# al-mcintyre/mCaller

Measured on NVIDIA B200. Metric: per-read site calls/sec, higher is better.
Workload: dtype f64

## Files before the change

include/mcaller_b200.h:

```cpp
#ifndef MCALLER_B200_H
#define MCALLER_B200_H

#include <stdint.h>

#ifdef __cplusplus
extern "C" {
#endif

#define MC_ABI_VERSION 3

#define MC_TILE_BYTES 3840
#define MC_TEXT_PAD 4096
#define MC_MAXK 8

enum {
    MC_OK = 0,
    MC_EINVAL = -1,
    MC_ECUDA = -2,
    MC_ECAPACITY = -3
};

typedef struct mc_refindex {
    int32_t n_contigs;
    int32_t k;
// ... 50 lines not shown

typedef struct mc_call {
    int64_t read_off;
    double prob;
    double feat[MC_MAXK + 1];
    int32_t read_len;
    int32_t mpos;
    int32_t site;
    uint32_t close_rec;
    uint16_t win_contig;
    uint16_t chrom_contig;
    uint8_t kind;
    uint8_t rev;
    uint8_t n_empty;
    uint8_t empty_mask;
    uint8_t model_sel;
    uint8_t label;
    uint8_t err;
    uint8_t pad0;
    uint32_t seg;
    uint32_t pad1;
    uint32_t pad2;
} mc_call;

enum { MC_CALL = 0, MC_TOO_MANY_SKIPS = 1, MC_MULTI_M = 2, MC_NONE = 3  };
#define MC_CE_CONTEXT 1u
#define MC_CE_MODELKEY 2u
#define MC_CE_BADNUM 4u
#define MC_CE_COLUMN 8u
#define MC_CE_SPACING 16u

enum { MC_MLP = 0, MC_LR = 1, MC_GNB = 2, MC_RF = 3 };
enum { MC_ACT_IDENTITY = 0, MC_ACT_LOGISTIC = 1, MC_ACT_TANH = 2, MC_ACT_RELU = 3 };
typedef struct mc_model {
    int32_t kind;
    int32_t n_in;
    int32_t n_layers;
    int32_t hidden_act;
    int32_t sizes[8];
    const double *d_weights;
    const double *d_biases;
    int32_t n_trees;
    int32_t max_nodes;
    const int32_t *d_tree_off;
    const int32_t *d_left;
    const int32_t *d_right;
    const int32_t *d_feature;
    const double *d_threshold;
    const double *d_leaf_p1;
} mc_model;

typedef struct mc_qual_entry {
    uint64_t hash;
    uint32_t check;
    uint32_t len;
    double qual;
} mc_qual_entry;


int mc_version(void);
int mc_sizeof(int what);
const char *mc_last_error(void);

int mc_read_u64(const uint64_t *d_src, int64_t n, uint64_t *h_dst, void *stream);

int mc_scan(const uint8_t *d_text, int64_t nbytes, const mc_refindex *ref, int dense,
            mc_record *d_rec, int64_t rec_cap, uint32_t *d_tile_tab , uint32_t *d_run_tab ,
            uint64_t *d_counters, void *stream);

int mc_scan_run_len(int64_t nbytes);

int mc_scan_set_run_len(int run_len);

int64_t mc_num_tiles(int64_t nbytes);

int64_t mc_workspace_bytes(int64_t n);

int mc_order_records(const uint8_t *d_text, int64_t nbytes, const mc_refindex *ref, const uint32_t *d_tile_tab, int64_t n_tiles,
                     uint32_t *d_run_tab, int run_len, const mc_record *d_rec_in, int64_t rec_in_cap, const uint64_t *d_scan_counters,
                     mc_record *d_rec_out, int64_t rec_out_cap, uint64_t *d_n_out, uint32_t *d_seg_flags ,
                     uint32_t *d_run_first , void *d_ws, void *stream);

int mc_segment_reads(const uint8_t *d_text, mc_record *d_rec, const uint64_t *d_n_records, int64_t rec_cap,
                     uint32_t *d_seg_flags , const uint32_t *d_run_first, int64_t n_runs,
                     uint32_t *d_seg_start, uint64_t *d_nseg, void *d_ws, void *stream);

int mc_segment_quality(const uint8_t *d_text, const mc_record *d_rec, const uint32_t *d_seg_start, const uint64_t *d_nseg,
                       int64_t seg_cap, const mc_qual_entry *d_table, int64_t table_size, double *d_seg_qual, uint64_t *d_err,
                       void *stream);

int mc_build_windows(const mc_record *d_rec, const uint64_t *d_n_records, int64_t rec_cap, const uint32_t *d_seg_start,
                     const uint64_t *d_nseg, int64_t seg_cap, const double *d_seg_qual, const mc_refindex *ref, int skip_thresh,
                     double qual_thresh, int two_models, mc_call *d_calls, int64_t call_cap, uint32_t *d_seg_count,
                     uint64_t *d_ncalls, void *d_ws, double *d_spill, int64_t spill_cap, void *stream);

typedef struct mc_carry {
    mc_call row;
    uint32_t valid;
    int32_t first_kept_contig;
    uint64_t chunks;
    uint64_t pad[6];
} mc_carry;
int mc_carry_reset(mc_carry *d_carry, void *stream);
int mc_carry_rows(mc_call *d_rows, const uint64_t *d_ncalls, const mc_record *d_rec, const uint64_t *d_n_records,
                  const uint32_t *d_seg_start, const uint64_t *d_nseg, const double *d_seg_qual, double qual_thresh,
                  mc_carry *d_carry, uint64_t *d_nrows_out, const uint64_t *d_abort, void *stream);
int mc_chunk_guard(const uint64_t *d_counters, int64_t rec_cap, const uint64_t *d_n_records, int64_t rec_out_cap,
                   const uint64_t *d_nseg, int64_t seg_cap, const uint64_t *d_ncalls, int64_t call_cap, uint64_t *d_abort,
                   uint64_t *d_sticky , void *stream);
int mc_carry_close(mc_carry *d_carry, int closing_contig, const int64_t *d_next_contigs, int from, int count, mc_call *d_row_out,
                   uint32_t *d_depth, uint32_t *d_meth, uint64_t *d_first, int64_t n_sites, uint64_t *d_row_base, void *stream);

int64_t mc_classify_workspace_bytes(int64_t row_cap);
int mc_classify(mc_call *d_calls, const uint64_t *d_nrows, int64_t row_cap, const mc_model *models, void *d_ws, void *stream);

int mc_hist_accumulate(const mc_call *d_calls, const uint64_t *d_nrows, int64_t row_cap, uint32_t *d_depth, uint32_t *d_meth,
                       uint64_t *d_first, int64_t n_sites, uint64_t *d_row_base, mc_call *d_odd, int64_t odd_cap, uint64_t *d_n_odd,
                       const uint64_t *d_abort , void *stream);

int mc_bed_select(const uint32_t *d_depth, const uint32_t *d_meth, int64_t n_sites, int64_t depth_thresh, double mod_thresh,
                  int control, uint8_t *d_flags, uint64_t *d_count, void *stream);

int mc_count_calls(const mc_call *d_calls, const uint64_t *d_nrows, int64_t row_cap, uint64_t *d_out, void *stream);

typedef struct mc_locus_entry {
    unsigned long long hash;
    unsigned long long first_off;
    unsigned long long check;
    uint32_t depth;
    uint32_t meth;
} mc_locus_entry;

typedef struct mc_diffs_row {
    uint64_t line_off;
    uint32_t slot;
    uint32_t values_off;
    uint32_t values_len;
    uint32_t prob_off;
    uint32_t prob_len;
    uint32_t pad;
} mc_diffs_row;
int mc_diffs_aggregate_ex(const uint8_t *d_text, int64_t nbytes, int64_t base_off, const uint64_t *d_posset, int64_t posset_size,
                          mc_locus_entry *d_table, int64_t table_size, uint64_t *d_counters, void *stream);
int mc_diffs_rehash(const mc_locus_entry *d_old, int64_t old_size, mc_locus_entry *d_table, int64_t table_size,
                    uint64_t *d_counters, void *stream);
int mc_diffs_rows(const uint8_t *d_text, int64_t nbytes, const uint64_t *d_posset, int64_t posset_size,
                  const mc_locus_entry *d_table, int64_t table_size, mc_diffs_row *d_rows, int64_t row_cap, uint64_t *d_nrows,
                  void *stream);
int mc_diffs_colstats(const uint8_t *d_text, const mc_diffs_row *d_rows, const uint32_t *d_order, int64_t n_rows,
                      const uint32_t *d_locus_off, int64_t n_loci, int ncols, double *d_vals, uint32_t *d_ncol,
                      double *d_stats, uint64_t *d_counters, void *stream);

int64_t mc_format_rows(const mc_call *h_calls, int64_t n_calls, const uint8_t *h_text, const uint8_t *carry_name,
                       int32_t carry_name_len, const char *const *contig_names, const char *const *marked_fwd,
                       const char *const *marked_rev, const int64_t *contig_len, int32_t n_contigs, int32_t k,
                       const char *base_label, const char *mod_label, int32_t with_prob, int32_t max_threads, char *out,
                       int64_t out_cap);

int64_t mc_fastq_tiles(int64_t nbytes);
int mc_fastq_index(const uint8_t *d_text, int64_t nbytes, uint32_t *d_tile_cnt, uint32_t *d_tile_off, uint64_t *d_line_start,
                   int64_t line_cap, uint64_t *d_n_newlines, void *d_ws, void *stream);
int mc_fastq_quality(const uint8_t *d_text, int64_t nbytes, const uint64_t *d_line_start, int64_t n_lines, mc_qual_entry *d_table,
                     int64_t table_size, uint32_t *d_owner, double *d_rec_mean, uint64_t *d_stats, void *stream);

#define MC_TRAIN_HIDDEN 100
#define MC_TRAIN_BATCH 200
typedef struct mc_train_job {
// ... 42 lines not shown
```

mcaller_b200/csrc/records.cu:

```cuda
#include "parse.cuh"

namespace {

constexpr int SCAN_THREADS = 256;
constexpr int SCAN_IPT = 8;
constexpr int SCAN_BLOCK = SCAN_THREADS * SCAN_IPT;

__global__ void __launch_bounds__(SCAN_THREADS) k_scan_reduce(const uint32_t *__restrict__ in, int64_t n_cap,
                                                            const unsigned long long *__restrict__ d_n,
                                                            unsigned long long *__restrict__ block_sums) {
    __shared__ int s_warp[SCAN_THREADS / 32 + 1];
    const int64_t n = d_n ? mc_dev_count(d_n, n_cap) : n_cap;
    const int64_t base = (int64_t)blockIdx.x * SCAN_BLOCK;
    unsigned long long acc = 0ull;
#pragma unroll
    for (int j = 0; j < SCAN_IPT; ++j) {
        const int64_t i = base + (int64_t)j * SCAN_THREADS + threadIdx.x;
        if (i < n) acc += in[i];
    }
    for (int d = 16; d > 0; d >>= 1) acc += __shfl_down_sync(0xffffffffu, acc, d);
    __shared__ unsigned long long s_sum[SCAN_THREADS / 32];
    if ((threadIdx.x & 31) == 0) s_sum[threadIdx.x >> 5] = acc;
    __syncthreads();
    if (threadIdx.x == 0) {
// ... 13 lines not shown
    const int lane = threadIdx.x & 31, wid = threadIdx.x >> 5;
    for (int64_t c0 = 0; c0 < nb; c0 += 1024) {
        const int64_t i = c0 + threadIdx.x;
        const unsigned long long v = (i < nb) ? block_sums[i] : 0ull;
        unsigned long long inc = v;
        for (int d = 1; d < 32; d <<= 1) {
            unsigned long long t = __shfl_up_sync(0xffffffffu, inc, d);
            if (lane >= d) inc += t;
        }
        if (lane == 31) s_w[wid] = inc;
        __syncthreads();
        if (wid == 0) {
            unsigned long long x = s_w[lane], xi = x;
            for (int d = 1; d < 32; d <<= 1) {
                unsigned long long t = __shfl_up_sync(0xffffffffu, xi, d);
                if (lane >= d) xi += t;
            }
            s_w[lane] = xi - x;
            if (lane == 31) s_w[32] = xi;
        }
        __syncthreads();
        const unsigned long long carry = s_carry;
        if (i < nb) block_sums[i] = carry + s_w[wid] + inc - v;
        __syncthreads();
        if (threadIdx.x == 0) s_carry = carry + s_w[32];
        __syncthreads();
    }
    if (threadIdx.x == 0 && d_total) *d_total = s_carry;
}

__global__ void __launch_bounds__(SCAN_THREADS) k_scan_down(const uint32_t *__restrict__ in, int64_t n_cap,
                                                          const unsigned long long *__restrict__ d_n,
                                                          const unsigned long long *__restrict__ block_sums,
                                                          uint32_t *__restrict__ out) {
    __shared__ int s_warp[SCAN_THREADS / 32 + 1];
    const int64_t n = d_n ? mc_dev_count(d_n, n_cap) : n_cap;
    if ((int64_t)blockIdx.x * SCAN_BLOCK >= n) return;
    const int64_t base = (int64_t)blockIdx.x * SCAN_BLOCK + (int64_t)threadIdx.x * SCAN_IPT;
    uint32_t v[SCAN_IPT];
    int sum = 0;
#pragma unroll
    for (int j = 0; j < SCAN_IPT; ++j) {
        const int64_t i = base + j;
        v[j] = (i < n) ? in[i] : 0u;
        sum += (int)v[j];
    }
    int total;
    int off = mc_block_exscan<SCAN_THREADS>(sum, s_warp, total);
    uint32_t run = (uint32_t)block_sums[blockIdx.x] + (uint32_t)off;
#pragma unroll
    for (int j = 0; j < SCAN_IPT; ++j) {
        const int64_t i = base + j;
        if (i < n) out[i] = run;
        run += v[j];
    }
}

}

int64_t mc_exscan_ws_bytes(int64_t n) { return ((n + SCAN_BLOCK - 1) / SCAN_BLOCK + 1) * 8 + 256; }

int mc_exscan_u32(const uint32_t *d_in, uint32_t *d_out, int64_t n_cap, const uint64_t *d_n, uint64_t *d_total, void *d_ws,
                  cudaStream_t st) {
    if (n_cap <= 0) {
        if (d_total) MC_CUDA_CHECK(cudaMemsetAsync(d_total, 0, 8, st));
        return MC_OK;
    }
    const int64_t nb = (n_cap + SCAN_BLOCK - 1) / SCAN_BLOCK;
    unsigned long long *sums = reinterpret_cast<unsigned long long *>(d_ws);
    const unsigned long long *dn = reinterpret_cast<const unsigned long long *>(d_n);
    k_scan_reduce<<<(unsigned)nb, SCAN_THREADS, 0, st>>>(d_in, n_cap, dn, sums);
    MC_LAUNCH_CHECK();
    k_scan_sums<<<1, 1024, 0, st>>>(sums, nb, reinterpret_cast<unsigned long long *>(d_total));
    MC_LAUNCH_CHECK();
    k_scan_down<<<(unsigned)nb, SCAN_THREADS, 0, st>>>(d_in, n_cap, dn, sums, d_out);
    MC_LAUNCH_CHECK();
    return MC_OK;
}

extern "C" int64_t mc_windows_workspace_bytes(int64_t rec_cap);
extern "C" int64_t mc_workspace_bytes(int64_t n) {
    if (n < 1) n = 1;
    const int64_t a = ((n * 4 + 255) / 256) * 256;
    const int64_t mine = 2 * a + mc_exscan_ws_bytes(n) + 512;
    const int64_t win = mc_windows_workspace_bytes(n);
    return mine > win ? mine : win;
}
static inline uint32_t *ws_a(void *ws) { return reinterpret_cast<uint32_t *>(ws); }
static inline uint32_t *ws_b(void *ws, int64_t n) { return reinterpret_cast<uint32_t *>(reinterpret_cast<uint8_t *>(ws) + ((n * 4 + 255) / 256) * 256); }
static inline void *ws_s(void *ws, int64_t n) { return reinterpret_cast<uint8_t *>(ws) + 2 * (((n * 4 + 255) / 256) * 256); }

namespace {

__global__ void __launch_bounds__(256) k_run_resolve(uint32_t *__restrict__ run_tab, int64_t n_runs, uint32_t *__restrict__ cnt_clean,
                                                    const unsigned long long *__restrict__ scan_counters, unsigned long long rec_in_cap) {
    const int64_t r = (int64_t)blockIdx.x * blockDim.x + threadIdx.x;
    if (r >= n_runs) return;
    if (scan_counters && (scan_counters[MC_C_OVERFLOW] != 0ull || scan_counters[MC_C_RECORDS] > rec_in_cap)) {
        cnt_clean[r] = 0u;
        return;
    }
    uint32_t count = run_tab[2 * r];
    const uint32_t v = run_tab[2 * r + 1];
    if (v & 1u) {
        int64_t p = r - 1;
        uint32_t st = 0u;
        while (p >= 0 && (st = (run_tab[2 * p + 1] >> 1) & 3u) == 0u) --p;
        if (p >= 0 && st == 1u && count > 0u) {
            run_tab[2 * r + 1] = v | 0x80000000u;
            --count;
        }
    }
    cnt_clean[r] = count;
}

__global__ void __launch_bounds__(256, 4) k_gather_finish(const uint8_t *__restrict__ text, int64_t limit, mc_refindex R,
                                                      const uint32_t *__restrict__ tile_tab, const uint32_t *__restrict__ run_tab,
                                                      const uint32_t *__restrict__ run_dst, int64_t n_tiles, int64_t n_runs, int run_len,
                                                      const mc_record *__restrict__ in, unsigned long long in_cap, mc_record *__restrict__ out,
                                                      unsigned long long out_cap, uint32_t *__restrict__ seg_flags,
                                                      uint32_t *__restrict__ run_first) {
    const int lane = threadIdx.x & 31;
    const int64_t warp0 = ((int64_t)blockIdx.x * blockDim.x + threadIdx.x) >> 5, n_warps = ((int64_t)gridDim.x * blockDim.x) >> 5;
    for (int64_t run = warp0; run < n_runs; run += n_warps) {
    const uint32_t rv = __ldg(run_tab + 2 * run + 1);
    const bool empty_run = __ldg(run_dst + run) == __ldg(run_dst + run + 1);
    if (run_first && lane == 0) run_first[run] = empty_run ? 0xFFFFFFFFu : __ldg(run_dst + run);
    if (__ldg(run_tab + 2 * run) == 0u) continue;
    const bool drop = (rv >> 31) != 0u;
    unsigned long long d_run = __ldg(run_dst + run);
    const int64_t c0 = run * run_len, c1 = min(c0 + (int64_t)run_len, n_tiles);
    long long carry_line = -1;
    uint32_t carry_span = 0u;
    for (int64_t cb = c0; cb < c1; cb += 32) {
        const int64_t c = cb + lane;
        unsigned long long src = 0ull;
        uint32_t cnt = 0u;
        if (c < c1) {
            const uint2 e = __ldg(reinterpret_cast<const uint2 *>(tile_tab) + c);
            src = e.x;
            cnt = e.y & 0xFFFFu;
            if (drop && ((e.y >> 16) & 1u) && cnt > 0u) { src += 1ull; --cnt; }
        }
        uint32_t incl = cnt;
#pragma unroll
        for (int d = 1; d < 32; d <<= 1) {
            const uint32_t t = __shfl_up_sync(0xffffffffu, incl, d);
            if (lane >= d) incl += t;
        }
        const uint32_t excl = incl - cnt, tot = __shfl_sync(0xffffffffu, incl, 31);
        for (uint32_t k0 = 0; k0 < tot; k0 += 32) {
            const uint32_t idx = k0 + lane;
            const bool act = idx < tot;
            int lo = 0, hi = 31;
#pragma unroll
            for (int st = 0; st < 5; ++st) {
                const int mid = (lo + hi + 1) >> 1;
                const uint32_t e_mid = __shfl_sync(0xffffffffu, excl, mid);
                if (e_mid <= idx) lo = mid; else hi = mid - 1;
            }
            const unsigned long long s_own = __shfl_sync(0xffffffffu, src, lo);
            const uint32_t e_own = __shfl_sync(0xffffffffu, excl, lo);
            const unsigned long long slot = s_own + (idx - e_own), dst = d_run + idx;
            const bool ok = act && slot < in_cap && dst < out_cap;
            alignas(16) mc_record r;
            long long line = -1;
            uint32_t span = 0u;
            if (ok) {
                const uint4 *sp = reinterpret_cast<const uint4 *>(in + slot);
                uint4 *dr = reinterpret_cast<uint4 *>(&r);
                dr[0] = __ldg(sp);
                dr[1] = __ldg(sp + 1);
                if (r.flags & MC_RF_RAW) mc_finish_record_win(text, limit, r);
                if (r.flags & MC_RF_CAND) {
                    const int cid = r.contig;
                    if (r.pos < __ldg(R.d_len + cid)) {
                        const int64_t g = __ldg(R.d_base + cid) + r.pos;
                        r.kbits_fwd = (uint8_t)mc_kmer_bits(R.d_site_fwd, g, R.k);
                        r.kbits_rev = (uint8_t)mc_kmer_bits(R.d_site_rev, g, R.k);
                    }
                }
                line = mc_rec_line(r);
                span = (uint32_t)r.name_off | ((uint32_t)r.name_len << 16);
            }
            long long pl = __shfl_up_sync(0xffffffffu, line, 1);
            uint32_t ps = __shfl_up_sync(0xffffffffu, span, 1);
            if (lane == 0) { pl = carry_line; ps = carry_span; }
            if (ok) {
                uint32_t sf = 1u;
                if (pl >= 0) {
                    uint32_t fl = r.flags | MC_RF_SEGKNOWN;
                    sf = 0u;
                    if ((ps >> 16) != r.name_len || bytes_differ(text + pl + (ps & 0xFFFFu), text + line + r.name_off, r.name_len)) {
                        fl |= MC_RF_NEWREAD;
                        sf = 1u;
                    }
                    r.flags = (uint8_t)fl;
                }
                if (seg_flags) seg_flags[dst] = sf;
                uint4 *dp = reinterpret_cast<uint4 *>(out + dst);
                const uint4 *sr = reinterpret_cast<const uint4 *>(&r);
                dp[0] = sr[0];
                dp[1] = sr[1];
            }
            const int last = (int)min(tot - k0, 32u) - 1;
            carry_line = __shfl_sync(0xffffffffu, line, last);
            carry_span = __shfl_sync(0xffffffffu, span, last);
        }
        d_run += tot;
    }
    }
}

__global__ void __launch_bounds__(256) k_seg_flags(const uint8_t *__restrict__ text, mc_record *__restrict__ rec, int64_t n_cap,
                                                  const unsigned long long *__restrict__ d_n, uint32_t *__restrict__ flags,
                                                  const uint32_t *__restrict__ known) {
    const int64_t n = mc_dev_count(d_n, n_cap);
    const int64_t i = (int64_t)blockIdx.x * blockDim.x + threadIdx.x;
    if (i >= n) return;
    if (known) {
        const uint32_t kf = known[i];
        if (kf < 2u) { flags[i] = kf; return; }
    }
    uint32_t f = 1u;
    const mc_record b = rec[i];
    if (b.flags & MC_RF_SEGKNOWN) {
        f = (b.flags & MC_RF_NEWREAD) ? 1u : 0u;
    } else {
        if (i > 0) {
            const mc_record a = rec[i - 1];
            if (a.name_len == b.name_len)
                f = bytes_differ(text + mc_rec_line(a) + a.name_off, text + mc_rec_line(b) + b.name_off, a.name_len) ? 1u : 0u;
        }
        rec[i].flags = (uint8_t)(b.flags | MC_RF_SEGKNOWN | (f ? MC_RF_NEWREAD : 0u));
    }
    flags[i] = f;
}

__global__ void __launch_bounds__(256) k_seg_fix(const uint8_t *__restrict__ text, mc_record *__restrict__ rec, const unsigned long long *__restrict__ d_n,
                                                int64_t n_cap, const uint32_t *__restrict__ run_first, int64_t n_runs, uint32_t *__restrict__ flags) {
    const int64_t run = (int64_t)blockIdx.x * blockDim.x + threadIdx.x;
    if (run >= n_runs) return;
    const uint32_t i = run_first[run];
    if (i == 0xFFFFFFFFu || (int64_t)i >= mc_dev_count(d_n, n_cap)) return;
    uint32_t f = 1u;
    const mc_record b = rec[i];
    if (i > 0u) {
        const mc_record a = rec[i - 1];
        if (a.name_len == b.name_len)
            f = bytes_differ(text + mc_rec_line(a) + a.name_off, text + mc_rec_line(b) + b.name_off, a.name_len) ? 1u : 0u;
    }
    rec[i].flags = (uint8_t)(b.flags | MC_RF_SEGKNOWN | (f ? MC_RF_NEWREAD : 0u));
    flags[i] = f;
}

__global__ void __launch_bounds__(256) k_seg_starts(const uint32_t *__restrict__ flags, const uint32_t *__restrict__ excl, int64_t n_cap,
                                                   const unsigned long long *__restrict__ d_n, uint32_t *__restrict__ seg_start,
                                                   const unsigned long long *__restrict__ d_nseg) {
    const int64_t n = mc_dev_count(d_n, n_cap);
    const int64_t i = (int64_t)blockIdx.x * blockDim.x + threadIdx.x;
    if (i < n && flags[i]) seg_start[excl[i]] = (uint32_t)i;
    if (i == 0) seg_start[*d_nseg] = (uint32_t)n;
}

__global__ void __launch_bounds__(256) k_seg_quality(const uint8_t *__restrict__ text, const mc_record *__restrict__ rec,
                                                    const uint32_t *__restrict__ seg_start, int64_t seg_cap,
                                                    const unsigned long long *__restrict__ d_nseg,
                                                    const mc_qual_entry *__restrict__ table, unsigned long long mask,
                                                    double *__restrict__ seg_qual, unsigned long long *__restrict__ d_err) {
    const int64_t n_seg = mc_dev_count(d_nseg, seg_cap);
    const int64_t s = (int64_t)blockIdx.x * blockDim.x + threadIdx.x;
    if (s >= n_seg) return;
    const mc_record r = rec[seg_start[s]];
    const mc_read_key key = mc_read_key_of(text + mc_rec_line(r) + r.name_off, r.name_len);
    double q = __longlong_as_double(0x7ff8000000000000ll);
    unsigned long long slot = key.hash & mask;
    for (unsigned long long probe = 0; probe <= mask; ++probe) {
        const mc_qual_entry e = table[slot];
        if (e.hash == 0ull) break;
        if (e.hash == key.hash && e.check == key.check && e.len == key.len) { q = e.qual; break; }
        slot = (slot + 1) & mask;
    }
    if (q != q) atomicAdd(d_err, 1ull);
    seg_qual[s] = q;
}

}

extern "C" int mc_order_records(const uint8_t *d_text, int64_t nbytes, const mc_refindex *ref, const uint32_t *d_tile_tab, int64_t n_tiles,
                                uint32_t *d_run_tab, int run_len, const mc_record *d_rec_in, int64_t rec_in_cap,
                                const uint64_t *d_scan_counters, mc_record *d_rec_out, int64_t rec_out_cap, uint64_t *d_n_out,
                                uint32_t *d_seg_flags, uint32_t *d_run_first, void *d_ws, void *stream) {
    MC_REQUIRE(!d_seg_flags == !d_run_first, "d_seg_flags and d_run_first go together");
    MC_REQUIRE(d_text && ref && d_tile_tab && d_run_tab && d_rec_in && d_rec_out && d_n_out && d_ws, "null pointer");
    MC_REQUIRE(run_len >= 1, "run length must be >= 1");
    cudaStream_t st = (cudaStream_t)stream;
    if (n_tiles <= 0) {
        MC_CUDA_CHECK(cudaMemsetAsync(d_n_out, 0, 8, st));
        return MC_OK;
    }
    const int64_t n_runs = (n_tiles + run_len - 1) / run_len;
    uint32_t *cnt = ws_a(d_ws), *dst = ws_b(d_ws, n_runs + 1);
    MC_CUDA_CHECK(cudaMemsetAsync(cnt + n_runs, 0, 4, st));
    k_run_resolve<<<(unsigned)((n_runs + 255) / 256), 256, 0, st>>>(d_run_tab, n_runs, cnt, reinterpret_cast<const unsigned long long *>(d_scan_counters),
                                                                   (unsigned long long)rec_in_cap);
    MC_LAUNCH_CHECK();
    int rc = mc_exscan_u32(cnt, dst, n_runs + 1, nullptr, d_n_out, ws_s(d_ws, n_runs + 1), st);
    if (rc) return rc;
    int64_t gf_blocks = (n_runs * 32 + 255) / 256;
    {
        int dev = 0, sms = 0;
        MC_CUDA_CHECK(cudaGetDevice(&dev));
        MC_CUDA_CHECK(cudaDeviceGetAttribute(&sms, cudaDevAttrMultiProcessorCount, dev));
        const int64_t resident = (int64_t)sms * 4;
        if (gf_blocks > resident) gf_blocks = resident;
    }
    k_gather_finish<<<(unsigned)gf_blocks, 256, 0, st>>>(d_text, nbytes + MC_TEXT_PAD - 64, *ref, d_tile_tab, d_run_tab, dst, n_tiles,
                                                                          n_runs, run_len, d_rec_in, (unsigned long long)rec_in_cap, d_rec_out,
                                                                          (unsigned long long)rec_out_cap, d_seg_flags, d_run_first);
    MC_LAUNCH_CHECK();
    return MC_OK;
}

extern "C" int mc_segment_reads(const uint8_t *d_text, mc_record *d_rec, const uint64_t *d_n_records, int64_t rec_cap,
                                uint32_t *d_seg_flags, const uint32_t *d_run_first, int64_t n_runs, uint32_t *d_seg_start, uint64_t *d_nseg,
                                void *d_ws, void *stream) {
    MC_REQUIRE(d_text && d_rec && d_n_records && d_seg_start && d_nseg && d_ws, "null pointer");
    cudaStream_t st = (cudaStream_t)stream;
    if (rec_cap <= 0) {
        MC_CUDA_CHECK(cudaMemsetAsync(d_nseg, 0, 8, st));
        MC_CUDA_CHECK(cudaMemsetAsync(d_seg_start, 0, 4, st));
        return MC_OK;
    }
    uint32_t *flags = ws_a(d_ws), *excl = ws_b(d_ws, rec_cap);
    const unsigned nb = (unsigned)((rec_cap + 255) / 256);
    const unsigned long long *dn = reinterpret_cast<const unsigned long long *>(d_n_records);
    if (d_seg_flags && d_run_first) {
        flags = d_seg_flags;
        if (n_runs > 0) k_seg_fix<<<(unsigned)((n_runs + 255) / 256), 256, 0, st>>>(d_text, d_rec, dn, rec_cap, d_run_first, n_runs, flags);
    } else {
        k_seg_flags<<<nb, 256, 0, st>>>(d_text, d_rec, rec_cap, dn, flags, nullptr);
    }
    MC_LAUNCH_CHECK();
    int rc = mc_exscan_u32(flags, excl, rec_cap, d_n_records, d_nseg, ws_s(d_ws, rec_cap), st);
    if (rc) return rc;
    k_seg_starts<<<nb, 256, 0, st>>>(flags, excl, rec_cap, dn, d_seg_start, reinterpret_cast<const unsigned long long *>(d_nseg));
    MC_LAUNCH_CHECK();
    return MC_OK;
}

extern "C" int mc_segment_quality(const uint8_t *d_text, const mc_record *d_rec, const uint32_t *d_seg_start, const uint64_t *d_nseg,
                                  int64_t seg_cap, const mc_qual_entry *d_table, int64_t table_size, double *d_seg_qual,
                                  uint64_t *d_err, void *stream) {
    MC_REQUIRE(d_text && d_rec && d_seg_start && d_nseg && d_table && d_seg_qual && d_err, "null pointer");
    MC_REQUIRE(table_size > 0 && (table_size & (table_size - 1)) == 0, "table size must be a power of two");
    if (seg_cap <= 0) return MC_OK;
    k_seg_quality<<<(unsigned)((seg_cap + 255) / 256), 256, 0, (cudaStream_t)stream>>>(
        d_text, d_rec, d_seg_start, seg_cap, reinterpret_cast<const unsigned long long *>(d_nseg), d_table,
        (unsigned long long)(table_size - 1), d_seg_qual, reinterpret_cast<unsigned long long *>(d_err));
    MC_LAUNCH_CHECK();
    return MC_OK;
}
```

mcaller_b200/engine.py:

```python
import ctypes as C

import numpy as np
import torch

from . import _lib
from ._lib import CALL_DTYPE, CARRY_BYTES, MC_C_COUNT, MC_TEXT_PAD, RECORD_DTYPE, check

C_LINES, C_KEPT, C_RECORDS, C_SHORT, C_UNKNOWN, C_NNN, C_BADPOS, C_LONGLINE, C_OVERFLOW = range(9)

S_NSEG, S_MISSING_QUAL, S_NCALLS, S_CALL_OVERFLOW, S_ABORT, S_NREC, S_NROWS = 16, 17, 18, 19, 20, 21, 22
S_STATS = 24
S_WORDS = 32
P_ROW_BASE, P_N_ODD, P_POISON = 0, 1, 2
SPILL_CAP = 1 << 22
ODD_CAP = 1 << 16


def require_cuda():
    if not torch.cuda.is_available():
        raise _lib.McallerCudaError("mcaller_b200 needs a CUDA device (B200, sm_100a); there is no CPU fallback")


class ChunkResult(object):
    __slots__ = ("n_calls", "n_records", "n_segments", "counters", "calls_dev", "missing_quality", "stats", "nbytes")
# ... 110 lines not shown
                                    C.c_void_p(self.d_depth.data_ptr()) if hist else None, C.c_void_p(self.d_meth.data_ptr()) if hist else None,
                                    C.c_void_p(self.d_first.data_ptr()) if hist else None, self.ref.n_sites,
                                    self._persist_ptr(P_ROW_BASE), self._sptr()))
        self.launches += 1
        if not fetch:
            return None
        return self.d_carry_out.cpu().numpy().view(CALL_DTYPE)

    def _default_rec_cap(self, nbytes, n_tiles):
        slack = 256 * min(n_tiles, 8192) + 4096
        return (nbytes // 24 + slack) if self.dense else (nbytes // 1024 + 2 * n_tiles + slack)

    def _caps(self, nbytes, n_tiles):
        slack = 256 * min(n_tiles, 8192) + 4096
        if self.rec_per_byte:
            rec_cap = int(self.rec_per_byte * nbytes * 1.25) + slack
            call_cap = int(self.call_per_byte * nbytes * 1.25) + 1024
            seg_cap = int(self.seg_per_byte * nbytes * 1.5) + 1024
        else:
            rec_cap = self._default_rec_cap(nbytes, n_tiles)
            call_cap = rec_cap // 8 + 1024
            seg_cap = rec_cap
        rec_cap = int(min(max(rec_cap, 1), 2 ** 32 - 2))
        return rec_cap, int(max(call_cap, 1)), int(min(max(seg_cap, 1), rec_cap))

    def run_chunk(self, d_text, nbytes, rec_cap=None, call_cap=None):
        L = self.L
        if d_text.numel() < nbytes + MC_TEXT_PAD:
            raise ValueError("text tensor lacks the MC_TEXT_PAD newline padding")
        res = ChunkResult()
        res.nbytes = nbytes
        n_tiles = int(L.mc_num_tiles(nbytes))
        slack = 256 * min(n_tiles, 8192) + 4096
        if rec_cap is None and call_cap is None:
            rec_cap, call_cap, seg_cap = self._caps(nbytes, n_tiles)
        else:
            d_rec, d_call, d_seg = self._caps(nbytes, n_tiles)
            rec_cap = int(min(max(rec_cap if rec_cap is not None else d_rec, 1), 2 ** 32 - 2))
            call_cap = int(max(call_cap if call_cap is not None else d_call, 1))
            seg_cap = int(min(d_seg, rec_cap))
        attempts = 0
        while True:
            cnt = self._launch_chunk(d_text, nbytes, n_tiles, rec_cap, call_cap, seg_cap)
            reserved, n_rec, n_calls, n_seg = int(cnt[C_RECORDS]), int(cnt[S_NREC]), int(cnt[S_NCALLS]), int(cnt[S_NSEG])
            if nbytes > 0:
                self.rec_per_byte = max(self.rec_per_byte, reserved / nbytes)
                self.call_per_byte = max(self.call_per_byte, n_calls / nbytes)
                self.seg_per_byte = max(self.seg_per_byte, n_seg / nbytes)
            if not cnt[S_ABORT]:
                break
            self.redone += 1
            attempts += 1
            if attempts > 6:
                raise _lib.McallerCudaError("chunk keeps overflowing its buffers (counters: %s)" % list(map(int, cnt[:MC_C_COUNT])))
            if cnt[C_OVERFLOW] or reserved > rec_cap:
                if rec_cap >= 2 ** 32 - 2:
                    raise _lib.McallerCudaError("chunk produces more than 2^32 records; use smaller chunks")
                rec_cap = int(min(max(reserved, rec_cap * 2 if cnt[C_OVERFLOW] and reserved <= rec_cap else 0) + slack, 2 ** 32 - 2))
                call_cap = max(call_cap, rec_cap // 8 + 1024)
            elif n_seg > seg_cap:
                seg_cap = min(n_seg + 1024, rec_cap)
            else:
                call_cap = n_calls + 1024
        if attempts:
            self.d_persist[P_POISON] = 0
        res.counters = {nm: int(cnt[i]) for i, nm in enumerate(_lib.COUNTER_NAMES)}
        res.n_records = n_rec
        res.n_segments = int(cnt[S_NSEG])
        res.missing_quality = int(cnt[S_MISSING_QUAL])
        res.n_calls = int(cnt[S_NROWS])
        res.calls_dev = self._bufs["calls"]
        v = cnt[S_STATS:S_STATS + 7]
        res.stats = dict(calls=int(v[0]), pending=int(v[1]), too_many_skips=int(v[2]), multi=int(v[3]), errors=int(v[4]), methylated=int(v[5]),
                         pending_too_many_skips=int(v[6]))
        return res

    def _launch_chunk(self, d_text, nbytes, n_tiles, rec_cap, call_cap, seg_cap, read_status=True):
        L, st = self.L, self._sptr()
        V = C.c_void_p
        tile_tab = self._buf("tile_tab", 8 * max(n_tiles, 1))
        run_len = max(int(L.mc_scan_run_len(nbytes)), 1)
        n_runs = max((n_tiles + run_len - 1) // run_len, 1)
        run_tab = self._buf("run_tab", 8 * n_runs)
        run_first = self._buf("run_first", 4 * n_runs)
        rec_a = self._buf("rec_a", 32 * rec_cap)
        rec_b = self._buf("rec_b", 32 * rec_cap)
        ws = self._buf("ws", L.mc_workspace_bytes(max(rec_cap, n_tiles)))
        seg_start = self._buf("seg_start", 4 * (rec_cap + 2))
        seg_flags = self._buf("seg_flags", 4 * rec_cap)
        seg_qual = self._buf("seg_qual", 8 * seg_cap)
        seg_count = self._buf("seg_count", 4 * seg_cap)
        calls = self._buf("calls", CALL_DTYPE.itemsize * (call_cap + 1))
        self.d_small.zero_()
        if self.scan_events is not None:
            e0, e1 = torch.cuda.Event(enable_timing=True), torch.cuda.Event(enable_timing=True)
            e0.record()
        check(L.mc_scan(V(d_text.data_ptr()), nbytes, self.ref.ref(), self.scan_mode, V(rec_a.data_ptr()), rec_cap,
                        V(tile_tab.data_ptr()), V(run_tab.data_ptr()), V(self.d_small.data_ptr()), st))
        if self.scan_events is not None:
            e1.record()
            self.scan_events.append((e0, e1))
        check(L.mc_order_records(V(d_text.data_ptr()), nbytes, self.ref.ref(), V(tile_tab.data_ptr()), n_tiles, V(run_tab.data_ptr()), run_len, V(rec_a.data_ptr()), rec_cap,
                                 V(self.d_small.data_ptr()), V(rec_b.data_ptr()), rec_cap, self._status_ptr(S_NREC), V(seg_flags.data_ptr()),
                                 V(run_first.data_ptr()), V(ws.data_ptr()), st))
        check(L.mc_segment_reads(V(d_text.data_ptr()), V(rec_b.data_ptr()), self._status_ptr(S_NREC), rec_cap, V(seg_flags.data_ptr()), V(run_first.data_ptr()),
                                 n_runs if n_tiles else 0, V(seg_start.data_ptr()),
                                 self._status_ptr(S_NSEG), V(ws.data_ptr()), st))
        check(L.mc_segment_quality(V(d_text.data_ptr()), V(rec_b.data_ptr()), V(seg_start.data_ptr()), self._status_ptr(S_NSEG), seg_cap,
                                   V(self.d_qual.data_ptr()), self.qual_table_size, V(seg_qual.data_ptr()), self._status_ptr(S_MISSING_QUAL), st))
        rows1 = V(calls.data_ptr() + CALL_DTYPE.itemsize)
        check(L.mc_build_windows(V(rec_b.data_ptr()), self._status_ptr(S_NREC), rec_cap, V(seg_start.data_ptr()), self._status_ptr(S_NSEG),
                                 seg_cap, V(seg_qual.data_ptr()), self.ref.ref(), self.skip_thresh, self.qual_thresh, self.two_models,
                                 rows1, call_cap, V(seg_count.data_ptr()), self._status_ptr(S_NCALLS), V(ws.data_ptr()),
                                 V(self.d_spill.data_ptr()), SPILL_CAP, st))
        check(L.mc_chunk_guard(V(self.d_small.data_ptr()), rec_cap, self._status_ptr(S_NREC), rec_cap, self._status_ptr(S_NSEG), seg_cap,
                               self._status_ptr(S_NCALLS), call_cap, self._status_ptr(S_ABORT), self._persist_ptr(P_POISON), st))
        check(L.mc_carry_rows(V(calls.data_ptr()), self._status_ptr(S_NCALLS), V(rec_b.data_ptr()), self._status_ptr(S_NREC),
                              V(seg_start.data_ptr()), self._status_ptr(S_NSEG), V(seg_qual.data_ptr()), self.qual_thresh,
                              V(self.d_carry.data_ptr()), self._status_ptr(S_NROWS), self._status_ptr(S_ABORT), st))
        self.launches += 1 + 5 + 5 + 1 + 7 + 2
        if self.models is not None:
            cls_ws = self._buf("cls_ws", L.mc_classify_workspace_bytes(call_cap + 1))
            check(L.mc_classify(V(calls.data_ptr()), self._status_ptr(S_NROWS), call_cap + 1, self.models.array, V(cls_ws.data_ptr()), st))
            self.launches += 2
            if self.histogram:
                check(L.mc_hist_accumulate(V(calls.data_ptr()), self._status_ptr(S_NROWS), call_cap + 1, V(self.d_depth.data_ptr()),
                                           V(self.d_meth.data_ptr()), V(self.d_first.data_ptr()), self.ref.n_sites, self._persist_ptr(P_ROW_BASE),
                                           V(self.d_odd.data_ptr()), ODD_CAP, self._persist_ptr(P_N_ODD), self._status_ptr(S_ABORT), st))
                self.launches += 2
        check(L.mc_count_calls(V(calls.data_ptr()), self._status_ptr(S_NROWS), call_cap + 1, self._status_ptr(S_STATS), st))
        self.launches += 1
        if not read_status:
            return None
        return self._read_status().copy()

    def launch_chunk(self, d_text, nbytes):
        if not self.rec_per_byte:
            raise _lib.McallerCudaError("launch_chunk needs a preceding run_chunk (capacities are learned from it)")
        n_tiles = int(self.L.mc_num_tiles(nbytes))
        rec_cap, call_cap, seg_cap = self._caps(nbytes, n_tiles)
        self._launch_chunk(d_text, nbytes, n_tiles, rec_cap, call_cap, seg_cap, read_status=False)

    def overflowed(self, clear=True):
        v = int(self.d_persist[P_POISON].item())
        if clear and v:
            self.d_persist[P_POISON] = 0
        return bool(v)

    def count_rows(self, res):
        return dict(res.stats)

    def records(self, n_rec):
        return self._bufs["rec_b"][: n_rec * 32].cpu().numpy().view(RECORD_DTYPE)

    def histogram_host(self):
        return (self.d_depth.cpu().numpy().view(np.uint32), self.d_meth.cpu().numpy().view(np.uint32),
                self.d_first.cpu().numpy().view(np.uint64))

    def bed_select(self, depth_thresh, mod_thresh, control=False):
        ns = max(self.ref.n_sites, 1)
        if getattr(self, "d_bed_flags", None) is None:
            self.d_bed_flags = torch.zeros(ns, dtype=torch.uint8, device=self.device)
            self.d_bed_count = torch.zeros(1, dtype=torch.int64, device=self.device)
        check(self.L.mc_bed_select(C.c_void_p(self.d_depth.data_ptr()), C.c_void_p(self.d_meth.data_ptr()), self.ref.n_sites, int(depth_thresh),
                                   float(mod_thresh), 1 if control else 0, C.c_void_p(self.d_bed_flags.data_ptr()),
                                   C.c_void_p(self.d_bed_count.data_ptr()), self._sptr()))
        self.launches += 1
        return self.d_bed_flags, self.d_bed_count

    def odd_rows(self):
        n = int(self.d_persist[P_N_ODD].item())
        if n > ODD_CAP:
            raise _lib.McallerCudaError("more than %d rows close on another contig than their window's" % ODD_CAP)
        return self.d_odd[: n * CALL_DTYPE.itemsize].cpu().numpy().view(CALL_DTYPE)
```

Baseline: 49.16 million.

## Split gather-finish into index pass and flat overlapping-tile finish kernel

The warp-per-run gather/finish kernel is replaced by two passes. The first writes only a destination-to-source index array. The second is a flat kernel where each warp handles 31 output records plus one overlap lane, so the name comparison with the previous record happens inside the warp using register shuffles rather than a serial carry. Segment starting points are now computed by a fused bitmask scan (reduce, sums, starts), which drops the run_first fixup kernel and the separate exclusive scan. This is meant to fix load imbalance across runs of uneven size and to cut launches, at the cost of an extra index array round trip through global memory and one redundantly loaded record per warp.

```diff
diff --git a/include/mcaller_b200.h b/include/mcaller_b200.h
--- a/include/mcaller_b200.h
+++ b/include/mcaller_b200.h
@@ -156,7 +156,7 @@
                      uint32_t *d_run_first , void *d_ws, void *stream);
 
 int mc_segment_reads(const uint8_t *d_text, mc_record *d_rec, const uint64_t *d_n_records, int64_t rec_cap,
-                     uint32_t *d_seg_flags , const uint32_t *d_run_first, int64_t n_runs,
+                     uint32_t *d_seg_flags , const uint32_t *d_run_first , int64_t n_runs,
                      uint32_t *d_seg_start, uint64_t *d_nseg, void *d_ws, void *stream);
 
 int mc_segment_quality(const uint8_t *d_text, const mc_record *d_rec, const uint32_t *d_seg_start, const uint64_t *d_nseg,
diff --git a/mcaller_b200/csrc/records.cu b/mcaller_b200/csrc/records.cu
--- a/mcaller_b200/csrc/records.cu
+++ b/mcaller_b200/csrc/records.cu
@@ -119,7 +119,7 @@
 extern "C" int64_t mc_workspace_bytes(int64_t n) {
     if (n < 1) n = 1;
     const int64_t a = ((n * 4 + 255) / 256) * 256;
-    const int64_t mine = 2 * a + mc_exscan_ws_bytes(n) + 512;
+    const int64_t mine = 3 * a + mc_exscan_ws_bytes(n) + 1024;
     const int64_t win = mc_windows_workspace_bytes(n);
     return mine > win ? mine : win;
 }
@@ -151,24 +151,16 @@
     cnt_clean[r] = count;
 }
 
-__global__ void __launch_bounds__(256, 4) k_gather_finish(const uint8_t *__restrict__ text, int64_t limit, mc_refindex R,
-                                                      const uint32_t *__restrict__ tile_tab, const uint32_t *__restrict__ run_tab,
-                                                      const uint32_t *__restrict__ run_dst, int64_t n_tiles, int64_t n_runs, int run_len,
-                                                      const mc_record *__restrict__ in, unsigned long long in_cap, mc_record *__restrict__ out,
-                                                      unsigned long long out_cap, uint32_t *__restrict__ seg_flags,
-                                                      uint32_t *__restrict__ run_first) {
+__global__ void __launch_bounds__(256) k_order_index(const uint32_t *__restrict__ tile_tab, const uint32_t *__restrict__ run_tab,
+                                                    const uint32_t *__restrict__ run_dst, int64_t n_tiles, int64_t n_runs, int run_len,
+                                                    unsigned long long in_cap, uint32_t *__restrict__ src_idx, unsigned long long out_cap) {
     const int lane = threadIdx.x & 31;
     const int64_t warp0 = ((int64_t)blockIdx.x * blockDim.x + threadIdx.x) >> 5, n_warps = ((int64_t)gridDim.x * blockDim.x) >> 5;
     for (int64_t run = warp0; run < n_runs; run += n_warps) {
-    const uint32_t rv = __ldg(run_tab + 2 * run + 1);
-    const bool empty_run = __ldg(run_dst + run) == __ldg(run_dst + run + 1);
-    if (run_first && lane == 0) run_first[run] = empty_run ? 0xFFFFFFFFu : __ldg(run_dst + run);
-    if (__ldg(run_tab + 2 * run) == 0u) continue;
-    const bool drop = (rv >> 31) != 0u;
     unsigned long long d_run = __ldg(run_dst + run);
+    if (d_run == __ldg(run_dst + run + 1)) continue;
+    const bool drop = (__ldg(run_tab + 2 * run + 1) >> 31) != 0u;
     const int64_t c0 = run * run_len, c1 = min(c0 + (int64_t)run_len, n_tiles);
-    long long carry_line = -1;
-    uint32_t carry_span = 0u;
     for (int64_t cb = c0; cb < c1; cb += 32) {
         const int64_t c = cb + lane;
         unsigned long long src = 0ull;
@@ -188,7 +180,6 @@
         const uint32_t excl = incl - cnt, tot = __shfl_sync(0xffffffffu, incl, 31);
         for (uint32_t k0 = 0; k0 < tot; k0 += 32) {
             const uint32_t idx = k0 + lane;
-            const bool act = idx < tot;
             int lo = 0, hi = 31;
 #pragma unroll
             for (int st = 0; st < 5; ++st) {
@@ -199,54 +190,99 @@
             const unsigned long long s_own = __shfl_sync(0xffffffffu, src, lo);
             const uint32_t e_own = __shfl_sync(0xffffffffu, excl, lo);
             const unsigned long long slot = s_own + (idx - e_own), dst = d_run + idx;
-            const bool ok = act && slot < in_cap && dst < out_cap;
-            alignas(16) mc_record r;
-            long long line = -1;
-            uint32_t span = 0u;
-            if (ok) {
-                const uint4 *sp = reinterpret_cast<const uint4 *>(in + slot);
-                uint4 *dr = reinterpret_cast<uint4 *>(&r);
-                dr[0] = __ldg(sp);
-                dr[1] = __ldg(sp + 1);
-                if (r.flags & MC_RF_RAW) mc_finish_record_win(text, limit, r);
-                if (r.flags & MC_RF_CAND) {
-                    const int cid = r.contig;
-                    if (r.pos < __ldg(R.d_len + cid)) {
-                        const int64_t g = __ldg(R.d_base + cid) + r.pos;
-                        r.kbits_fwd = (uint8_t)mc_kmer_bits(R.d_site_fwd, g, R.k);
-                        r.kbits_rev = (uint8_t)mc_kmer_bits(R.d_site_rev, g, R.k);
-                    }
+            if (idx < tot && dst < out_cap) src_idx[dst] = slot < in_cap ? (uint32_t)slot : 0xFFFFFFFFu;
+        }
+        d_run += tot;
+    }
+    }
+}
+
+constexpr int NAME_REG_BYTES = 64;
+__device__ __forceinline__ uint32_t name_differs_from_prev_lane(const uint8_t *p, int len) {
+    const uintptr_t ua = reinterpret_cast<uintptr_t>(p);
+    const uint4 *q = reinterpret_cast<const uint4 *>(ua & ~(uintptr_t)15);
+    const int sh = (int)(ua & 15), qw = sh >> 2, rb = 8 * (sh & 3);
+    const int n16 = len > 0 ? (sh + len + 15) >> 4 : 0;
+    uint4 cur = n16 > 0 ? __ldg(q) : make_uint4(0u, 0u, 0u, 0u);
+    uint32_t diff = 0u;
+#pragma unroll
+    for (int c = 0; c < NAME_REG_BYTES / 16; ++c) {
+        const uint4 nxt = c + 1 < n16 ? __ldg(q + c + 1) : make_uint4(0u, 0u, 0u, 0u);
+        const uint32_t v[8] = {cur.x, cur.y, cur.z, cur.w, nxt.x, nxt.y, nxt.z, nxt.w};
+        uint32_t s[5];
+#pragma unroll
+        for (int i = 0; i < 5; ++i) s[i] = qw == 0 ? v[i] : qw == 1 ? v[i + 1] : qw == 2 ? v[i + 2] : v[i + 3];
+#pragma unroll
+        for (int i = 0; i < 4; ++i) {
+            uint32_t w = __funnelshift_r(s[i], s[i + 1], rb);
+            const int left = len - 16 * c - 4 * i;
+            if (left < 4) w &= left <= 0 ? 0u : (1u << (8 * left)) - 1u;
+            diff |= w ^ __shfl_up_sync(0xffffffffu, w, 1);
+        }
+        cur = nxt;
+    }
+    return diff;
+}
+
+constexpr int FIN_TILE = 31;
+#ifndef MC_FIN_THREADS
+#define MC_FIN_THREADS 256
+#endif
+#ifndef MC_FIN_MIN_CTAS
+#define MC_FIN_MIN_CTAS 5
+#endif
+constexpr int FIN_THREADS = MC_FIN_THREADS;
+constexpr int FIN_MIN_CTAS = MC_FIN_MIN_CTAS;
+__global__ void __launch_bounds__(FIN_THREADS, FIN_MIN_CTAS) k_finish_records(const uint8_t *__restrict__ text, int64_t limit, mc_refindex R,
+                                                                      const uint32_t *__restrict__ src_idx, const mc_record *__restrict__ in,
+                                                                      unsigned long long in_cap, mc_record *__restrict__ out, int64_t out_cap,
+                                                                      const unsigned long long *__restrict__ d_n, uint32_t *__restrict__ seg_flags) {
+    const int64_t n = mc_dev_count(d_n, out_cap);
+    const int lane = threadIdx.x & 31;
+    const int64_t d0 = (((int64_t)blockIdx.x * blockDim.x + threadIdx.x) >> 5) * FIN_TILE;
+    if (d0 >= n) return;
+    const int64_t d = d0 + lane - 1;
+    alignas(16) mc_record r;
+    bool ok = false;
+    long long line = -1;
+    uint32_t span = 0u;
+    if (d >= 0 && d < n) {
+        const uint32_t slot = __ldg(src_idx + d);
+        if (slot < in_cap) {
+            ok = true;
+            const uint4 *sp = reinterpret_cast<const uint4 *>(in + slot);
+            uint4 *dr = reinterpret_cast<uint4 *>(&r);
+            dr[0] = __ldg(sp);
+            dr[1] = __ldg(sp + 1);
+            if (r.flags & MC_RF_RAW) mc_finish_record_win(text, limit, r);
+            if (lane > 0 && (r.flags & MC_RF_CAND)) {
+                const int cid = r.contig;
+                if (r.pos < __ldg(R.d_len + cid)) {
+                    const int64_t g = __ldg(R.d_base + cid) + r.pos;
+                    r.kbits_fwd = (uint8_t)mc_kmer_bits(R.d_site_fwd, g, R.k);
+                    r.kbits_rev = (uint8_t)mc_kmer_bits(R.d_site_rev, g, R.k);
                 }
-                line = mc_rec_line(r);
-                span = (uint32_t)r.name_off | ((uint32_t)r.name_len << 16);
             }
-            long long pl = __shfl_up_sync(0xffffffffu, line, 1);
-            uint32_t ps = __shfl_up_sync(0xffffffffu, span, 1);
-            if (lane == 0) { pl = carry_line; ps = carry_span; }
-            if (ok) {
-                uint32_t sf = 1u;
-                if (pl >= 0) {
-                    uint32_t fl = r.flags | MC_RF_SEGKNOWN;
-                    sf = 0u;
-                    if ((ps >> 16) != r.name_len || bytes_differ(text + pl + (ps & 0xFFFFu), text + line + r.name_off, r.name_len)) {
-                        fl |= MC_RF_NEWREAD;
-                        sf = 1u;
-                    }
-                    r.flags = (uint8_t)fl;
-                }
-                if (seg_flags) seg_flags[dst] = sf;
-                uint4 *dp = reinterpret_cast<uint4 *>(out + dst);
-                const uint4 *sr = reinterpret_cast<const uint4 *>(&r);
-                dp[0] = sr[0];
-                dp[1] = sr[1];
-            }
-            const int last = (int)min(tot - k0, 32u) - 1;
-            carry_line = __shfl_sync(0xffffffffu, line, last);
-            carry_span = __shfl_sync(0xffffffffu, span, last);
-        }
-        d_run += tot;
-    }
-    }
+            line = mc_rec_line(r);
+            span = (uint32_t)r.name_off | ((uint32_t)r.name_len << 16);
+        }
+    }
+    const long long pl = __shfl_up_sync(0xffffffffu, line, 1);
+    const uint32_t ps = __shfl_up_sync(0xffffffffu, span, 1);
+    const bool reg_name = ok && r.name_len <= NAME_REG_BYTES;
+    const uint32_t name_diff = name_differs_from_prev_lane(reg_name ? text + line + r.name_off : text, reg_name ? r.name_len : 0);
+    if (lane == 0 || !ok) return;
+    uint32_t sf = 1u;
+    if (pl >= 0 && (ps >> 16) == r.name_len) {
+        sf = reg_name ? (name_diff != 0u ? 1u : 0u)
+                      : (bytes_differ(text + pl + (ps & 0xFFFFu), text + line + r.name_off, r.name_len) ? 1u : 0u);
+    }
+    r.flags = (uint8_t)(r.flags | MC_RF_SEGKNOWN | (sf ? MC_RF_NEWREAD : 0u));
+    if (seg_flags) seg_flags[d] = sf;
+    uint4 *dp = reinterpret_cast<uint4 *>(out + d);
+    const uint4 *sr = reinterpret_cast<const uint4 *>(&r);
+    dp[0] = sr[0];
+    dp[1] = sr[1];
 }
 
 __global__ void __launch_bounds__(256) k_seg_flags(const uint8_t *__restrict__ text, mc_record *__restrict__ rec, int64_t n_cap,
@@ -274,30 +310,31 @@
     flags[i] = f;
 }
 
-__global__ void __launch_bounds__(256) k_seg_fix(const uint8_t *__restrict__ text, mc_record *__restrict__ rec, const unsigned long long *__restrict__ d_n,
-                                                int64_t n_cap, const uint32_t *__restrict__ run_first, int64_t n_runs, uint32_t *__restrict__ flags) {
-    const int64_t run = (int64_t)blockIdx.x * blockDim.x + threadIdx.x;
-    if (run >= n_runs) return;
-    const uint32_t i = run_first[run];
-    if (i == 0xFFFFFFFFu || (int64_t)i >= mc_dev_count(d_n, n_cap)) return;
-    uint32_t f = 1u;
-    const mc_record b = rec[i];
-    if (i > 0u) {
-        const mc_record a = rec[i - 1];
-        if (a.name_len == b.name_len)
-            f = bytes_differ(text + mc_rec_line(a) + a.name_off, text + mc_rec_line(b) + b.name_off, a.name_len) ? 1u : 0u;
-    }
-    rec[i].flags = (uint8_t)(b.flags | MC_RF_SEGKNOWN | (f ? MC_RF_NEWREAD : 0u));
-    flags[i] = f;
-}
-
-__global__ void __launch_bounds__(256) k_seg_starts(const uint32_t *__restrict__ flags, const uint32_t *__restrict__ excl, int64_t n_cap,
-                                                   const unsigned long long *__restrict__ d_n, uint32_t *__restrict__ seg_start,
-                                                   const unsigned long long *__restrict__ d_nseg) {
+__global__ void __launch_bounds__(SCAN_THREADS) k_seg_starts(const uint32_t *__restrict__ flags, int64_t n_cap,
+                                                           const unsigned long long *__restrict__ d_n,
+                                                           const unsigned long long *__restrict__ tile_first,
+                                                           uint32_t *__restrict__ seg_start, const unsigned long long *__restrict__ d_nseg) {
+    __shared__ int s_warp[SCAN_THREADS / 32 + 1];
     const int64_t n = mc_dev_count(d_n, n_cap);
-    const int64_t i = (int64_t)blockIdx.x * blockDim.x + threadIdx.x;
-    if (i < n && flags[i]) seg_start[excl[i]] = (uint32_t)i;
-    if (i == 0) seg_start[*d_nseg] = (uint32_t)n;
+    if (blockIdx.x == 0 && threadIdx.x == 0) seg_start[*d_nseg] = (uint32_t)n;
+    if ((int64_t)blockIdx.x * SCAN_BLOCK >= n) return;
+    const int64_t base = (int64_t)blockIdx.x * SCAN_BLOCK + (int64_t)threadIdx.x * SCAN_IPT;
+    static_assert(SCAN_IPT == 8, "two 16-byte loads per thread");
+    uint32_t m = 0u;
+    if (base + SCAN_IPT <= n) {
+        const uint4 *p = reinterpret_cast<const uint4 *>(flags + base);
+        const uint4 u = p[0], v = p[1];
+        m = (u.x != 0u) | (u.y != 0u) << 1 | (u.z != 0u) << 2 | (u.w != 0u) << 3 | (v.x != 0u) << 4 | (v.y != 0u) << 5 |
+            (v.z != 0u) << 6 | (v.w != 0u) << 7;
+    } else {
+        for (int j = 0; j < SCAN_IPT && base + j < n; ++j) m |= (flags[base + j] != 0u) << j;
+    }
+    int total;
+    uint32_t o = (uint32_t)tile_first[blockIdx.x] + (uint32_t)mc_block_exscan<SCAN_THREADS>(__popc(m), s_warp, total);
+    while (m) {
+        seg_start[o++] = (uint32_t)(base + __ffs(m) - 1);
+        m &= m - 1u;
+    }
 }
 
 __global__ void __launch_bounds__(256) k_seg_quality(const uint8_t *__restrict__ text, const mc_record *__restrict__ rec,
@@ -328,7 +365,7 @@
                                 uint32_t *d_run_tab, int run_len, const mc_record *d_rec_in, int64_t rec_in_cap,
                                 const uint64_t *d_scan_counters, mc_record *d_rec_out, int64_t rec_out_cap, uint64_t *d_n_out,
                                 uint32_t *d_seg_flags, uint32_t *d_run_first, void *d_ws, void *stream) {
-    MC_REQUIRE(!d_seg_flags == !d_run_first, "d_seg_flags and d_run_first go together");
+    (void)d_run_first;
     MC_REQUIRE(d_text && ref && d_tile_tab && d_run_tab && d_rec_in && d_rec_out && d_n_out && d_ws, "null pointer");
     MC_REQUIRE(run_len >= 1, "run length must be >= 1");
     cudaStream_t st = (cudaStream_t)stream;
@@ -337,24 +374,32 @@
         return MC_OK;
     }
     const int64_t n_runs = (n_tiles + run_len - 1) / run_len;
-    uint32_t *cnt = ws_a(d_ws), *dst = ws_b(d_ws, n_runs + 1);
+    uint32_t *src_idx = ws_a(d_ws);
+    void *ws_runs = ws_b(d_ws, rec_out_cap);
+    uint32_t *cnt = ws_a(ws_runs), *dst = ws_b(ws_runs, n_runs + 1);
     MC_CUDA_CHECK(cudaMemsetAsync(cnt + n_runs, 0, 4, st));
     k_run_resolve<<<(unsigned)((n_runs + 255) / 256), 256, 0, st>>>(d_run_tab, n_runs, cnt, reinterpret_cast<const unsigned long long *>(d_scan_counters),
                                                                    (unsigned long long)rec_in_cap);
     MC_LAUNCH_CHECK();
-    int rc = mc_exscan_u32(cnt, dst, n_runs + 1, nullptr, d_n_out, ws_s(d_ws, n_runs + 1), st);
+    int rc = mc_exscan_u32(cnt, dst, n_runs + 1, nullptr, d_n_out, ws_s(ws_runs, n_runs + 1), st);
     if (rc) return rc;
-    int64_t gf_blocks = (n_runs * 32 + 255) / 256;
+    int64_t idx_blocks = (n_runs * 32 + 255) / 256;
     {
-        int dev = 0, sms = 0;
+        int dev = 0, sms = 0, per_sm = 0;
         MC_CUDA_CHECK(cudaGetDevice(&dev));
         MC_CUDA_CHECK(cudaDeviceGetAttribute(&sms, cudaDevAttrMultiProcessorCount, dev));
-        const int64_t resident = (int64_t)sms * 4;
-        if (gf_blocks > resident) gf_blocks = resident;
-    }
-    k_gather_finish<<<(unsigned)gf_blocks, 256, 0, st>>>(d_text, nbytes + MC_TEXT_PAD - 64, *ref, d_tile_tab, d_run_tab, dst, n_tiles,
-                                                                          n_runs, run_len, d_rec_in, (unsigned long long)rec_in_cap, d_rec_out,
-                                                                          (unsigned long long)rec_out_cap, d_seg_flags, d_run_first);
+        MC_CUDA_CHECK(cudaOccupancyMaxActiveBlocksPerMultiprocessor(&per_sm, k_order_index, 256, 0));
+        const int64_t resident = (int64_t)sms * (per_sm > 0 ? per_sm : 1);
+        if (idx_blocks > resident) idx_blocks = resident;
+    }
+    k_order_index<<<(unsigned)idx_blocks, 256, 0, st>>>(d_tile_tab, d_run_tab, dst, n_tiles, n_runs, run_len, (unsigned long long)rec_in_cap,
+                                                         src_idx, (unsigned long long)rec_out_cap);
+    MC_LAUNCH_CHECK();
+    const int64_t fin_warps = (rec_out_cap + FIN_TILE - 1) / FIN_TILE;
+    if (fin_warps == 0) return MC_OK;
+    k_finish_records<<<(unsigned)((fin_warps * 32 + FIN_THREADS - 1) / FIN_THREADS), FIN_THREADS, 0, st>>>(
+        d_text, nbytes + MC_TEXT_PAD - 64, *ref, src_idx, d_rec_in, (unsigned long long)rec_in_cap, d_rec_out, rec_out_cap,
+        reinterpret_cast<const unsigned long long *>(d_n_out), d_seg_flags);
     MC_LAUNCH_CHECK();
     return MC_OK;
 }
@@ -362,6 +407,8 @@
 extern "C" int mc_segment_reads(const uint8_t *d_text, mc_record *d_rec, const uint64_t *d_n_records, int64_t rec_cap,
                                 uint32_t *d_seg_flags, const uint32_t *d_run_first, int64_t n_runs, uint32_t *d_seg_start, uint64_t *d_nseg,
                                 void *d_ws, void *stream) {
+    (void)d_run_first;
+    (void)n_runs;
     MC_REQUIRE(d_text && d_rec && d_n_records && d_seg_start && d_nseg && d_ws, "null pointer");
     cudaStream_t st = (cudaStream_t)stream;
     if (rec_cap <= 0) {
@@ -369,19 +416,20 @@
         MC_CUDA_CHECK(cudaMemsetAsync(d_seg_start, 0, 4, st));
         return MC_OK;
     }
-    uint32_t *flags = ws_a(d_ws), *excl = ws_b(d_ws, rec_cap);
-    const unsigned nb = (unsigned)((rec_cap + 255) / 256);
     const unsigned long long *dn = reinterpret_cast<const unsigned long long *>(d_n_records);
-    if (d_seg_flags && d_run_first) {
-        flags = d_seg_flags;
-        if (n_runs > 0) k_seg_fix<<<(unsigned)((n_runs + 255) / 256), 256, 0, st>>>(d_text, d_rec, dn, rec_cap, d_run_first, n_runs, flags);
-    } else {
-        k_seg_flags<<<nb, 256, 0, st>>>(d_text, d_rec, rec_cap, dn, flags, nullptr);
-    }
-    MC_LAUNCH_CHECK();
-    int rc = mc_exscan_u32(flags, excl, rec_cap, d_n_records, d_nseg, ws_s(d_ws, rec_cap), st);
-    if (rc) return rc;
-    k_seg_starts<<<nb, 256, 0, st>>>(flags, excl, rec_cap, dn, d_seg_start, reinterpret_cast<const unsigned long long *>(d_nseg));
+    uint32_t *flags = d_seg_flags;
+    if (!flags) {
+        flags = ws_a(d_ws);
+        k_seg_flags<<<(unsigned)((rec_cap + 255) / 256), 256, 0, st>>>(d_text, d_rec, rec_cap, dn, flags, nullptr);
+        MC_LAUNCH_CHECK();
+    }
+    const int64_t nb = (rec_cap + SCAN_BLOCK - 1) / SCAN_BLOCK;
+    unsigned long long *tile_first = reinterpret_cast<unsigned long long *>(ws_s(d_ws, rec_cap));
+    k_scan_reduce<<<(unsigned)nb, SCAN_THREADS, 0, st>>>(flags, rec_cap, dn, tile_first);
+    MC_LAUNCH_CHECK();
+    k_scan_sums<<<1, 1024, 0, st>>>(tile_first, nb, reinterpret_cast<unsigned long long *>(d_nseg));
+    MC_LAUNCH_CHECK();
+    k_seg_starts<<<(unsigned)nb, SCAN_THREADS, 0, st>>>(flags, rec_cap, dn, tile_first, d_seg_start, reinterpret_cast<const unsigned long long *>(d_nseg));
     MC_LAUNCH_CHECK();
     return MC_OK;
 }
diff --git a/mcaller_b200/engine.py b/mcaller_b200/engine.py
--- a/mcaller_b200/engine.py
+++ b/mcaller_b200/engine.py
@@ -216,7 +216,6 @@
         run_len = max(int(L.mc_scan_run_len(nbytes)), 1)
         n_runs = max((n_tiles + run_len - 1) // run_len, 1)
         run_tab = self._buf("run_tab", 8 * n_runs)
-        run_first = self._buf("run_first", 4 * n_runs)
         rec_a = self._buf("rec_a", 32 * rec_cap)
         rec_b = self._buf("rec_b", 32 * rec_cap)
         ws = self._buf("ws", L.mc_workspace_bytes(max(rec_cap, n_tiles)))
@@ -236,8 +235,8 @@
             self.scan_events.append((e0, e1))
         check(L.mc_order_records(V(d_text.data_ptr()), nbytes, self.ref.ref(), V(tile_tab.data_ptr()), n_tiles, V(run_tab.data_ptr()), run_len, V(rec_a.data_ptr()), rec_cap,
                                  V(self.d_small.data_ptr()), V(rec_b.data_ptr()), rec_cap, self._status_ptr(S_NREC), V(seg_flags.data_ptr()),
-                                 V(run_first.data_ptr()), V(ws.data_ptr()), st))
-        check(L.mc_segment_reads(V(d_text.data_ptr()), V(rec_b.data_ptr()), self._status_ptr(S_NREC), rec_cap, V(seg_flags.data_ptr()), V(run_first.data_ptr()),
+                                 None, V(ws.data_ptr()), st))
+        check(L.mc_segment_reads(V(d_text.data_ptr()), V(rec_b.data_ptr()), self._status_ptr(S_NREC), rec_cap, V(seg_flags.data_ptr()), None,
                                  n_runs if n_tiles else 0, V(seg_start.data_ptr()),
                                  self._status_ptr(S_NSEG), V(ws.data_ptr()), st))
         check(L.mc_segment_quality(V(d_text.data_ptr()), V(rec_b.data_ptr()), V(seg_start.data_ptr()), self._status_ptr(S_NSEG), seg_cap,
@@ -252,7 +251,7 @@
         check(L.mc_carry_rows(V(calls.data_ptr()), self._status_ptr(S_NCALLS), V(rec_b.data_ptr()), self._status_ptr(S_NREC),
                               V(seg_start.data_ptr()), self._status_ptr(S_NSEG), V(seg_qual.data_ptr()), self.qual_thresh,
                               V(self.d_carry.data_ptr()), self._status_ptr(S_NROWS), self._status_ptr(S_ABORT), st))
-        self.launches += 1 + 5 + 5 + 1 + 7 + 2
+        self.launches += 1 + 6 + 3 + 1 + 7 + 2
         if self.models is not None:
             cls_ws = self._buf("cls_ws", L.mc_classify_workspace_bytes(call_cap + 1))
             check(L.mc_classify(V(calls.data_ptr()), self._status_ptr(S_NROWS), call_cap + 1, self.models.array, V(cls_ws.data_ptr()), st))
```

Result: faster. 50.16 million, median of 6 (+2.0%).
